# Alexander-H-Liu/End-to-end-ASR-Pytorch

Hardware: AMD Instinct MI355X
Metric: audio frames/sec training (LAS+CTC, LibriSpeech 80-mel) (higher is better)
Workload: dtype f32; 1 GPU; cfg3: {"B": 32, "T": 1600, "D": 80, "V": 5000, "L": 64}; global_batch=32, parallelism=dp1

## Files before the change

### end-to-end-asr-pytorch_amd/csrc/core.cpp

```cpp
#include "common.h"
#include "knobs.h"
#include <cstdlib>
#include <mutex>
#include <vector>

namespace {
struct DevInfo {
    int cu_count = 0;
    int lds_per_cu = 0;
    bool ok = false;
};
DevInfo g_dev[64];

struct ProfRec {
    hipEvent_t a, b;
    int id;
};
bool g_prof_on = false;
std::vector<ProfRec> g_pending;
double g_total_ms[PROF_NUM];
int64_t g_launches[PROF_NUM];
std::mutex g_mu;
hipEvent_t g_cur[PROF_NUM];
}

namespace {
AsrkKnobs g_knobs;
std::once_flag g_knobs_once;
int env_int(const char *name) {
    const char *e = getenv(name);
    return e ? atoi(e) : AsrkKnobs::UNSET;
}
int env_present(const char *name) { return getenv(name) ? 1 : AsrkKnobs::UNSET; }
void read_knobs() {
    AsrkKnobs &k = g_knobs;
    k.gemm_noskinny = env_present("ASRK_GEMM_NOSKINNY");
    k.skinny_sk = env_int("ASRK_SKINNY_SK");
    k.gemm_dbg = env_int("ASRK_GEMM_DBG");
    k.gemm_nofast = env_present("ASRK_GEMM_NOFAST");
    k.split_w256 = env_int("ASRK_SPLIT_W256");
    k.split_tail = env_int("ASRK_SPLIT_TAIL");
    k.split_mfma = env_int("ASRK_SPLIT_MFMA");
    k.fwd_mt = env_int("ASRK_FWD_MT");
    k.fwd_nt = env_int("ASRK_FWD_NT");
    k.rec_bf_mt4 = env_int("ASRK_REC_BF_MT4");
    k.bwd_ub = env_int("ASRK_BWD_UB");
    k.bwd_nt = env_int("ASRK_BWD_NT");
    k.fwd_poll = env_int("ASRK_FWD_POLL");
    k.fwd_presleep = env_int("ASRK_FWD_PRESLEEP");
    k.bwd_poll = env_int("ASRK_BWD_POLL");
    k.bwd_presleep = env_int("ASRK_BWD_PRESLEEP");
    k.dbg_noload = env_present("ASRK_DBG_NOLOAD");
    k.deterministic = env_int("ASRK_DETERMINISTIC");
}
}

const AsrkKnobs &asrk_knobs_() {
    std::call_once(g_knobs_once, read_knobs);
    return g_knobs;
}

extern "C" int asrk_version(void) { return 200; }

extern "C" const char *asrk_strerror(int rc) {
    switch (rc) {
        case ASRK_OK: return "ok";
        case ASRK_EINVAL: return "asrk: invalid argument";
        case ASRK_ESHAPE: return "asrk: shape not supported by the persistent gfx950 kernels";
        case ASRK_EWORKSPACE: return "asrk: workspace too small";
        case ASRK_EDEVICE: return "asrk: device lacks the CUs/LDS the persistent kernel needs";
        case ASRK_ETIMEOUT: return "asrk: in-kernel grid synchronisation timed out";
        default: break;
    }
    if (rc > 0) return hipGetErrorString((hipError_t)rc);
    return "asrk: unknown error";
}

extern "C" int asrk_init(int device) {
    if (device < 0 || device >= 64) return ASRK_EINVAL;
    (void)asrk_knobs_();
    if (!g_dev[device].ok) {
        hipDeviceProp_t prop;
        hipError_t e = hipGetDeviceProperties(&prop, device);
        if (e != hipSuccess) return (int)e > 0 ? -(1000 + (int)e) : ASRK_EDEVICE;
        g_dev[device].cu_count = prop.multiProcessorCount;
        g_dev[device].lds_per_cu = (int)prop.maxSharedMemoryPerMultiProcessor;
        g_dev[device].ok = true;
    }
    return g_dev[device].cu_count;
}

extern "C" int asrk_cu_count_(void) {
    int dev = 0;
    if (hipGetDevice(&dev) != hipSuccess) return 0;
    if (dev < 0 || dev >= 64) return 0;
    if (!g_dev[dev].ok) {
        if (asrk_init(dev) <= 0) return 0;
    }
    return g_dev[dev].cu_count;
}

static double g_work[PROF_NUM] = {0};

static unsigned g_prof_mask = 0xffffffffu;
extern "C" void asrk_profile_enable(int on) { g_prof_on = on != 0; }
extern "C" void asrk_profile_families(unsigned mask) { g_prof_mask = mask; }
static inline bool prof_live(int id) { return g_prof_on && id >= 0 && id < PROF_NUM && ((g_prof_mask >> id) & 1u); }

extern "C" void asrk_profile_reset(void) {
    std::lock_guard<std::mutex> lk(g_mu);
    for (auto &r : g_pending) {
        hipEventDestroy(r.a);
        hipEventDestroy(r.b);
    }
    g_pending.clear();
    for (int i = 0; i < PROF_NUM; ++i) {
        g_total_ms[i] = 0.0;
        g_launches[i] = 0;
        g_work[i] = 0.0;
    }
}

extern "C" void asrk_prof_work_(int id, double flops) {
    if (prof_live(id)) g_work[id] += flops;
}
extern "C" int asrk_profile_get_work(int id, double *flops) {
    if (id < 0 || id >= PROF_NUM || !flops) return ASRK_EINVAL;
    *flops = g_work[id];
    return ASRK_OK;
}

extern "C" void asrk_prof_begin_(int id, hipStream_t s) {
    if (!prof_live(id)) return;
    hipEvent_t a;
    if (hipEventCreate(&a) != hipSuccess) return;
    hipEventRecord(a, s);
    g_cur[id] = a;
}

extern "C" void asrk_prof_end_(int id, hipStream_t s) {
    if (!prof_live(id)) return;
    hipEvent_t b;
    if (hipEventCreate(&b) != hipSuccess) return;
    hipEventRecord(b, s);
    std::lock_guard<std::mutex> lk(g_mu);
    g_pending.push_back({g_cur[id], b, id});
}

extern "C" void asrk_prof_launches_(int id, int64_t n) {
    if (!prof_live(id)) return;
    std::lock_guard<std::mutex> lk(g_mu);
    g_launches[id] += n;
}

extern "C" int asrk_profile_get(int id, double *total_ms, int64_t *launches) {
    if (id < 0 || id >= PROF_NUM) return ASRK_EINVAL;
    std::lock_guard<std::mutex> lk(g_mu);
    for (auto &r : g_pending) {
        hipEventSynchronize(r.b);
        float ms = 0.f;
        if (hipEventElapsedTime(&ms, r.a, r.b) == hipSuccess) {
            g_total_ms[r.id] += ms;
            g_launches[r.id] += 1;
        }
        hipEventDestroy(r.a);
        hipEventDestroy(r.b);
    }
    g_pending.clear();
    if (total_ms) *total_ms = g_total_ms[id];
    if (launches) *launches = g_launches[id];
    return ASRK_OK;
}
```

### end-to-end-asr-pytorch_amd/csrc/gemm_split.hip

```cpp
#include "common.h"
#include "knobs.h"
#include <algorithm>
#include <climits>

extern "C" int asrk_cu_count_(void);

namespace {

typedef __bf16 bf16x8 __attribute__((ext_vector_type(8)));

constexpr int PIECE = 1024;

struct SplitGemmArgs {
    const unsigned char *Ap, *Bp;
    float *C;
    const float *bias, *bias2;
    int M, N, ldc;
    int KC;
    size_t rb_stride_a, rb_stride_b;
    int nk;
    int tiles_m, tiles_n;
    float alpha, beta;
    int slices, ldw;
    float *ws;
};

__device__ __forceinline__ void split8(const float (&v)[8], u32x4 (&w)[3]) {
    unsigned h[3][8];
#pragma unroll
    for (int e = 0; e < 8; ++e) {
        const float a = v[e];
        const __bf16 b0 = (__bf16)a;
        const float r1 = a - (float)b0;
        const __bf16 b1 = (__bf16)r1;
        const float r2 = r1 - (float)b1;
        const __bf16 b2 = (__bf16)r2;
        h[0][e] = __builtin_bit_cast(unsigned short, b0);
        h[1][e] = __builtin_bit_cast(unsigned short, b1);
        h[2][e] = __builtin_bit_cast(unsigned short, b2);
    }
#pragma unroll
    for (int p = 0; p < 3; ++p)
#pragma unroll
        for (int q = 0; q < 4; ++q) w[p][q] = h[p][2 * q] | (h[p][2 * q + 1] << 16);
}

template <bool VEC>
__global__ __launch_bounds__(256) void split_panel_kernel(const float *__restrict__ src, int ld, int R, int K,
                                                          unsigned char *__restrict__ dst, int KC, int RB,
                                                          size_t rb_stride) {
    constexpr int CHUNK = 3 * PIECE;
    const int lane = threadIdx.x & 63;
    const int KG = KC >> 2;
    const int64_t item = (int64_t)blockIdx.x * 4 + (threadIdx.x >> 6);
    if (item >= (int64_t)RB * KG) return;
    const int rb = (int)(item / KG), c0 = (int)(item - (int64_t)rb * KG) * 4;
    unsigned char *drb = dst + (size_t)rb * rb_stride;
    const int c = c0 + (lane & 3), k0 = c * 8;
#pragma unroll
    for (int it = 0; it < 4; ++it) {
        const int rl = it * 16 + (lane >> 2), row = rb * 64 + rl;
        float v[8];
        const float *s = src + (size_t)row * ld + k0;
        if (VEC && row < R && k0 + 8 <= K) {
            const f32x4 lo = *reinterpret_cast<const f32x4 *>(s), hi = *reinterpret_cast<const f32x4 *>(s + 4);
            v[0] = lo[0]; v[1] = lo[1]; v[2] = lo[2]; v[3] = lo[3];
            v[4] = hi[0]; v[5] = hi[1]; v[6] = hi[2]; v[7] = hi[3];
        } else {
#pragma unroll
            for (int e = 0; e < 8; ++e) v[e] = (row < R && k0 + e < K) ? s[e] : 0.f;
        }
        u32x4 w[3];
        split8(v, w);
        unsigned char *d = drb + (size_t)c * CHUNK + rl * 16;
#pragma unroll
        for (int p = 0; p < 3; ++p) *reinterpret_cast<u32x4 *>(d + p * PIECE) = w[p];
    }
}

template <int NCG>
__global__ __launch_bounds__(256) void split_panel_t_kernel(const float *__restrict__ src, int ld, int R, int K,
                                                            unsigned char *__restrict__ dst, int KC, int RB,
                                                            size_t rb_stride) {
    constexpr int CHUNK = 3 * PIECE;
    const int lane = threadIdx.x & 63, wave = __builtin_amdgcn_readfirstlane(threadIdx.x >> 6);
    const int64_t item = (int64_t)blockIdx.x * 4 + wave;
    const int KGn = KC / NCG;
    if (item >= (int64_t)RB * KGn) return;
    const int g = (int)(item / RB), rb = (int)(item - (int64_t)g * RB);
    const int c0 = g * NCG, k0 = c0 * 8, row = rb * 64 + lane;
    float v[NCG][8];
    const float *s = src + (size_t)k0 * ld + row;
    if (k0 + 8 * NCG <= K && rb * 64 + 64 <= R) {
#pragma unroll
        for (int cc = 0; cc < NCG; ++cc)
#pragma unroll
            for (int e = 0; e < 8; ++e) v[cc][e] = s[(size_t)(cc * 8 + e) * ld];
    } else {
#pragma unroll
        for (int cc = 0; cc < NCG; ++cc)
#pragma unroll
            for (int e = 0; e < 8; ++e)
                v[cc][e] = (row < R && k0 + cc * 8 + e < K) ? s[(size_t)(cc * 8 + e) * ld] : 0.f;
    }
    unsigned char *d = dst + (size_t)rb * rb_stride + (size_t)c0 * CHUNK + lane * 16;
#pragma unroll
    for (int cc = 0; cc < NCG; ++cc) {
        u32x4 w[3];
        split8(v[cc], w);
#pragma unroll
        for (int p = 0; p < 3; ++p) *reinterpret_cast<u32x4 *>(d + (size_t)cc * CHUNK + p * PIECE) = w[p];
    }
}

template <int N>
__device__ __forceinline__ void glds16_run(const unsigned char *g, unsigned voff, unsigned char *l) {
    static_assert(N >= 1 && N <= 4, "immediate offset range");
    const auto *gp = (const __attribute__((address_space(1))) unsigned char *)g + voff;
    auto *lp = (__attribute__((address_space(3))) void *)l;
    __builtin_amdgcn_global_load_lds(gp, lp, 16, 0, 0);
    if constexpr (N > 1) __builtin_amdgcn_global_load_lds(gp, lp, 16, PIECE, 0);
    if constexpr (N > 2) __builtin_amdgcn_global_load_lds(gp, lp, 16, 2 * PIECE, 0);
    if constexpr (N > 3) __builtin_amdgcn_global_load_lds(gp, lp, 16, 3 * PIECE, 0);
}

template <int N>
__device__ __forceinline__ void wait_vm() {
    static_assert(N >= 0 && N < 64, "vmcnt is a 6-bit field");
    __builtin_amdgcn_s_waitcnt((N & 15) | 0x70 | 0xF00 | (((N >> 4) & 3) << 14));
}
__device__ __forceinline__ void wait_lgkm0() { __builtin_amdgcn_s_waitcnt(0xC07F); }

template <int NC, int NST, bool SPEC, int WM, bool SK = false>
__global__ __launch_bounds__(SPEC ? (WM == 2 ? 512 : 704) : 256) void gemm_bf16x6_kernel(SplitGemmArgs p) {
    extern __shared__ __attribute__((aligned(1024))) unsigned char lds[];
    static_assert(WM == 2 || (WM == 4 && SPEC), "256-row tiles only with DMA waves");
    static_assert(!SK || NST >= 2, "the split-K epilogue transposes through a stage the last k-tile does not use");
    constexpr int NPL = 3, CHUNK = NPL * PIECE;
    constexpr int NCW = 2 * WM;
    constexpr int NRG = WM + 2;
    constexpr int RPD = WM == 2 ? 1 : 2;
    constexpr int REGION = NC * CHUNK;
    constexpr int STAGE = NRG * REGION;
    constexpr int LPT = NC * NPL * RPD;
    const int tid = threadIdx.x, lane = tid & 63;
    const int wave = __builtin_amdgcn_readfirstlane(tid >> 6);
    const int ntiles = p.tiles_m * p.tiles_n;
    const int slice = SK ? blockIdx.x / ntiles : 0, bid = SK ? blockIdx.x - slice * ntiles : blockIdx.x;
    const int kt0 = SK ? (int)((long)slice * p.nk / p.slices) : 0;
    const int nk = SK ? (int)((long)(slice + 1) * p.nk / p.slices) - kt0 : p.nk;
    const int q8 = ntiles >> 3, r8 = ntiles & 7, xcd = bid & 7, loc = bid >> 3;
    const int tile = (xcd < r8 ? xcd * (q8 + 1) : r8 * (q8 + 1) + (xcd - r8) * q8) + loc;
    constexpr int BAND = 8;
    const int band = tile / (BAND * p.tiles_m);
    const int band_w = min(BAND, p.tiles_n - band * BAND);
    const int in_band = tile - band * BAND * p.tiles_m;
    const int tm = in_band / band_w, tn = band * BAND + in_band % band_w;

    const bool loader = !SPEC || wave >= NCW, worker = !SPEC || wave < NCW;
    const int wr = worker ? wave >> 1 : 0, wc = wave & 1;
    const int ltm = tm, ltn = tn;
    const int r0 = (SPEC ? wave - NCW : wave) * RPD;
    const unsigned char *gsrc[RPD];
#pragma unroll
    for (int q = 0; q < RPD; ++q) {
        const int r = r0 + q;
        gsrc[q] = (r < WM ? p.Ap + (size_t)(ltm * WM + r) * p.rb_stride_a
                          : p.Bp + (size_t)(ltn * 2 + r - WM) * p.rb_stride_b);
        if (SK) gsrc[q] += (size_t)kt0 * REGION;
    }
    const unsigned voff = lane * 16;
    unsigned char *ldst = lds + r0 * REGION;
    static_assert((NC * NPL) % 4 == 0, "a region is issued as runs of four pieces");
    auto issue = [&](int kt, int stage) {
        unsigned char *l = ldst + stage * STAGE;
#pragma unroll
        for (int q = 0; q < RPD; ++q) {
// ... 247 lines not shown
            if (++stage == NST) stage = 0;
        }
        return;
    }

    const int wr = wave >> 1, wc = wave & 1;
    f32x16 acc[2][4];
#pragma unroll
    for (int i = 0; i < 2; ++i)
#pragma unroll
        for (int j = 0; j < 4; ++j)
#pragma unroll
            for (int r = 0; r < 16; ++r) acc[i][j][r] = 0.f;
    const int frag_off = ((lane >> 5) * NPL) * PIECE + (lane & 31) * 16;
    const unsigned char *abase = lds + wr * REGION + frag_off;
    const unsigned char *bbase = lds + (2 + wc * 2) * REGION + frag_off;
    bf16x8 fa1[2], fa2[2], fb1[4], fb2[4], fa0[2][2], fb0[2][4];
    auto rd_a1 = [&](bf16x8 &dst, int stage, int pl, int i) {
        dst = *reinterpret_cast<const bf16x8 *>(abase + stage * STAGE + pl * PIECE + i * 512);
    };
    auto rd_b1 = [&](bf16x8 &dst, int stage, int pl, int j) {
        dst = *reinterpret_cast<const bf16x8 *>(bbase + stage * STAGE + (j >> 1) * REGION + pl * PIECE + (j & 1) * 512);
    };
    auto rd_a = [&](bf16x8 (&dst)[2], int stage, int pl) {
#pragma unroll
        for (int i = 0; i < 2; ++i) rd_a1(dst[i], stage, pl, i);
    };
    auto rd_b = [&](bf16x8 (&dst)[4], int stage, int pl) {
#pragma unroll
        for (int j = 0; j < 4; ++j) rd_b1(dst[j], stage, pl, j);
    };
#define ASRK_TERM8(FA, FB)                                                                                 \
    do {                                                                                                   \
        _Pragma("unroll") for (int i = 0; i < 2; ++i) _Pragma("unroll") for (int j = 0; j < 4; ++j)         \
            acc[i][j] = __builtin_amdgcn_mfma_f32_32x32x16_bf16(FA[i], FB[j], acc[i][j], 0, 0, 0);          \
        __builtin_amdgcn_sched_barrier(0);                                                                 \
    } while (0)
#define ASRK_TERM8_RD(FA, FB, RD)                                                                          \
    do {                                                                                                   \
        _Pragma("unroll") for (int m = 0; m < 8; ++m) {                                                    \
            acc[m >> 2][m & 3] =                                                                           \
                __builtin_amdgcn_mfma_f32_32x32x16_bf16(FA[m >> 2], FB[m & 3], acc[m >> 2][m & 3], 0, 0, 0); \
            __builtin_amdgcn_sched_barrier(0);                                                             \
            RD(m);                                                                                         \
            __builtin_amdgcn_sched_barrier(0);                                                             \
        }                                                                                                  \
    } while (0)
#define ASRK_STEP(P)                                                                                       \
    do {                                                                                                   \
        int nstage = stage + 1;                                                                            \
        if (nstage == NST) nstage = 0;                                                                     \
        ASRK_TERM8(fa2, fb0[P]);                                                                           \
        wait_lgkm0();                                                                                      \
        __builtin_amdgcn_s_barrier();                                           \
        auto rd2 = [&](int m) {                                                                            \
            if (m == 0) rd_a1(fa2[0], nstage, 2, 0);                                                       \
            else if (m == 2) rd_a1(fa2[1], nstage, 2, 1);                                                  \
            else if (m == 4) rd_b1(fb0[1 - (P)][0], nstage, 0, 0);                                         \
            else if (m == 6) rd_b1(fb0[1 - (P)][1], nstage, 0, 1);                                         \
        };                                                                                                 \
        ASRK_TERM8_RD(fa0[P], fb2, rd2);                                                                   \
        auto rd3 = [&](int m) {                                                                            \
            if ((m & 1) == 0) rd_b1(fb2[m >> 1], nstage, 2, m >> 1);                                       \
        };                                                                                                 \
        ASRK_TERM8_RD(fa0[P], fb1, rd3);                                                                   \
        auto rd4 = [&](int m) {                                                                            \
            if (m == 0) rd_b1(fb0[1 - (P)][2], nstage, 0, 2);                                              \
            else if (m == 2) rd_b1(fb0[1 - (P)][3], nstage, 0, 3);                                         \
            else if (m == 4) rd_a1(fa0[1 - (P)][0], nstage, 0, 0);                                         \
            else if (m == 6) rd_a1(fa0[1 - (P)][1], nstage, 0, 1);                                         \
        };                                                                                                 \
        ASRK_TERM8_RD(fa1, fb1, rd4);                                                                      \
        auto rd5 = [&](int m) {                                                                            \
            if ((m & 1) == 0) rd_b1(fb1[m >> 1], nstage, 1, m >> 1);                                       \
        };                                                                                                 \
        ASRK_TERM8_RD(fa1, fb0[P], rd5);                                                                   \
        auto rd6 = [&](int m) {                                                                            \
            if (m == 1) rd_a1(fa1[0], nstage, 1, 0);                                                       \
            else if (m == 4) rd_a1(fa1[1], nstage, 1, 1);                                                  \
        };                                                                                                 \
        ASRK_TERM8_RD(fa0[P], fb0[P], rd6);                                                                \
        stage = nstage;                                                                                    \
    } while (0)

    __builtin_amdgcn_s_barrier();
    rd_a(fa2, 0, 2); rd_b(fb0[0], 0, 0); rd_a(fa0[0], 0, 0); rd_b(fb2, 0, 2); rd_b(fb1, 0, 1); rd_a(fa1, 0, 1);
    int stage = 0;
    for (int kt = 0; kt < nk; kt += 2) {
        ASRK_STEP(0);
        ASRK_STEP(1);
    }
#undef ASRK_STEP
#undef ASRK_TERM8_RD
#undef ASRK_TERM8

    const int row0 = tm * 128 + wr * 64 + 4 * (lane >> 5), col0 = tn * 256 + wc * 128 + (lane & 31);
#pragma unroll
    for (int j = 0; j < 4; ++j) {
        const int col = col0 + j * 32;
        if (col >= p.N) continue;
        float bsum = 0.f;
        if (p.bias) bsum += p.bias[col];
        if (p.bias2) bsum += p.bias2[col];
#pragma unroll
        for (int i = 0; i < 2; ++i)
#pragma unroll
            for (int r = 0; r < 16; ++r) {
                const int row = row0 + i * 32 + (r & 3) + 8 * (r >> 2);
                if (row >= p.M) continue;
                float *c = p.C + (size_t)row * p.ldc + col;
                float v = p.alpha * acc[i][j][r] + bsum;
                if (p.beta != 0.f) v += p.beta * *c;
                *c = v;
            }
    }
}

template <int NST, int NDW>
int launch_split_gemm_w256(const SplitGemmArgs &a, int rb_b, hipStream_t s) {
    constexpr int lds = NST * 6 * 2 * 3 * PIECE;
    auto kern = gemm_bf16x6_w256_kernel<NST, NDW>;
    static AsrkLdsLatch latch;
    ASRK_HIP(asrk_max_lds_once(latch, reinterpret_cast<const void *>(kern), lds));
    const int band = 2;
    hipLaunchKernelGGL(kern, dim3(a.tiles_m * a.tiles_n), dim3((4 + NDW) * 64), lds, s, a, rb_b, band);
    ASRK_LAUNCH_CHECK();
    return ASRK_OK;
}

#define ASRK_P16(FA, FB, ACC, RD)                                                                          \
    do {                                                                                                   \
        _Pragma("unroll") for (int m = 0; m < 16; ++m) {                                                   \
            ACC[m >> 2][m & 3] =                                                                           \
                __builtin_amdgcn_mfma_f32_16x16x32_bf16(FA[m >> 2], FB[m & 3], ACC[m >> 2][m & 3], 0, 0, 0); \
            __builtin_amdgcn_sched_barrier(0);                                                             \
            RD(m);                                                                                         \
            __builtin_amdgcn_sched_barrier(0);                                                             \
        }                                                                                                  \
    } while (0)

template <int START, int STRIDE>
__device__ __forceinline__ void rd16_at(int m, bf16x8 (&slot)[4], const unsigned char *src) {
    static_assert(START + 3 * STRIDE < 16, "inside one product");
    const int i = (m - START) / STRIDE;
    if (m >= START && i < 4 && START + i * STRIDE == m) slot[i] = *reinterpret_cast<const bf16x8 *>(src + i * 256);
}
__device__ __forceinline__ void rd16_all(bf16x8 (&slot)[4], const unsigned char *src) {
#pragma unroll
    for (int i = 0; i < 4; ++i) slot[i] = *reinterpret_cast<const bf16x8 *>(src + i * 256);
}

template <int P> struct StepSet { static constexpr int value = P; };

template <bool SK>
__global__ __launch_bounds__(512) void gemm_bf16x6_m16_kernel(SplitGemmArgs p) {
    extern __shared__ __attribute__((aligned(1024))) unsigned char lds[];
    constexpr int NPL = 3, NC = 4, NST = 3, CHUNK = NPL * PIECE;
    constexpr int REGION = NC * CHUNK, STAGE = 4 * REGION, LPT = NC * NPL;
    const int tid = threadIdx.x, lane = tid & 63;
    const int wave = __builtin_amdgcn_readfirstlane(tid >> 6);
    const int ntiles = p.tiles_m * p.tiles_n;
    const int slice = SK ? blockIdx.x / ntiles : 0, bid = SK ? blockIdx.x - slice * ntiles : blockIdx.x;
    const int kt0 = SK ? (int)((long)slice * p.nk / p.slices) : 0;
    const int nk = SK ? (int)((long)(slice + 1) * p.nk / p.slices) - kt0 : p.nk;
    const int q8 = ntiles >> 3, r8 = ntiles & 7, xcd = bid & 7, loc = bid >> 3;
    const int tile = (xcd < r8 ? xcd * (q8 + 1) : r8 * (q8 + 1) + (xcd - r8) * q8) + loc;
    constexpr int BAND = 8;
    const int band = tile / (BAND * p.tiles_m);
    const int band_w = min(BAND, p.tiles_n - band * BAND);
    const int in_band = tile - band * BAND * p.tiles_m;
    const int tm = in_band / band_w, tn = band * BAND + in_band % band_w;

    const bool worker = wave < 4;
    const int wr = worker ? wave >> 1 : 0, wc = wave & 1;
    const int r0 = worker ? 0 : wave - 4;
    const unsigned char *gsrc = (r0 < 2 ? p.Ap + (size_t)(tm * 2 + r0) * p.rb_stride_a
                                        : p.Bp + (size_t)(tn * 2 + r0 - 2) * p.rb_stride_b) + (size_t)kt0 * REGION;
    const unsigned voff = lane * 16;
    unsigned char *ldst = lds + r0 * REGION;
    auto issue = [&](int kt, int stage) {
        const unsigned char *g = gsrc + (size_t)kt * REGION;
        unsigned char *l = ldst + stage * STAGE;
#pragma unroll
        for (int j = 0; j < LPT; j += 4) glds16_run<4>(g + j * PIECE, voff, l + j * PIECE);
    };

    f32x4 acc[4][4];
#pragma unroll
    for (int i = 0; i < 4; ++i)
#pragma unroll
        for (int j = 0; j < 4; ++j)
#pragma unroll
            for (int r = 0; r < 4; ++r) acc[i][j][r] = 0.f;
    const int frag_off = ((lane >> 4) * NPL) * PIECE + (lane & 15) * 16;
    const unsigned char *abase = lds + wr * REGION + frag_off;
    const unsigned char *bbase = lds + (2 + wc) * REGION + frag_off;
    bf16x8 fa0[2][4], fa1[4], fa2[4], fb0[4], fb1[4], fb2[4];

    if (!worker) {
#pragma unroll
        for (int s = 0; s < NST; ++s)
            if (s < nk) issue(s, s);
        const int later = min(NST - 1, nk - 1);
        if (later >= 2) wait_vm<2 * LPT>();
        else if (later == 1) wait_vm<LPT>();
        else wait_vm<0>();
    }
    __builtin_amdgcn_s_barrier();
    if (worker) {
        rd16_all(fa0[0], abase); rd16_all(fb2, bbase + 2 * PIECE);
        rd16_all(fa1, abase + PIECE); rd16_all(fb1, bbase + PIECE); rd16_all(fa2, abase + 2 * PIECE);
        __builtin_amdgcn_sched_barrier(0);
    }

    int stage = 0, kt = 0;
    auto step = [&](auto set) {
        constexpr int P = decltype(set)::value, Q = 1 - P;
        int nstage = stage + 1;
        if (nstage == NST) nstage = 0;
        const unsigned char *bc = bbase + stage * STAGE;
        const unsigned char *an = abase + nstage * STAGE, *bn = bbase + nstage * STAGE;
        if (worker) {
            auto rd1 = [&](int m) { rd16_at<0, 4>(m, fb0, bc); };
            ASRK_P16(fa0[P], fb2, acc, rd1);
            auto rd2 = [&](int) {};
            ASRK_P16(fa1, fb1, acc, rd2);
            wait_lgkm0();
        } else {
            if (nk - 2 - kt >= 1) wait_vm<LPT>();
            else wait_vm<0>();
        }
        __builtin_amdgcn_s_barrier();
        if (worker) {
            auto rd3 = [&](int m) { rd16_at<0, 4>(m, fb2, bn + 2 * PIECE); };
            ASRK_P16(fa0[P], fb1, acc, rd3);
            auto rd4 = [&](int m) { rd16_at<0, 4>(m, fa0[Q], an); };
            ASRK_P16(fa2, fb0, acc, rd4);
            auto rd5 = [&](int m) { rd16_at<0, 4>(m, fa2, an + 2 * PIECE); rd16_at<2, 4>(m, fb1, bn + PIECE); };
            ASRK_P16(fa1, fb0, acc, rd5);
            auto rd6 = [&](int m) { rd16_at<0, 2>(m, fa1, an + PIECE); };
            ASRK_P16(fa0[P], fb0, acc, rd6);
        } else if (kt + NST < nk) {
            issue(kt + NST, stage);
        }
        stage = nstage;
        ++kt;
    };
    while (kt < nk) {
        step(StepSet<0>());
        if (kt < nk) step(StepSet<1>());
    }
    if (!worker) return;

    if constexpr (SK) {
        constexpr int PITCH = 68;
        static_assert(4 * 16 * PITCH * 4 <= STAGE, "transposition images fit one stage");
        float *img = reinterpret_cast<float *>(lds) + wave * 16 * PITCH;
        float *wsl = p.ws + (size_t)slice * p.M * p.ldw;
        const int wrow0 = tm * 128 + wr * 64, wcol0 = tn * 128 + wc * 64;
        wait_lgkm0();
#pragma unroll
        for (int i = 0; i < 4; ++i) {
#pragma unroll
            for (int j = 0; j < 4; ++j)
#pragma unroll
                for (int r = 0; r < 4; ++r) img[(4 * (lane >> 4) + r) * PITCH + j * 16 + (lane & 15)] = acc[i][j][r];
            __builtin_amdgcn_fence(__ATOMIC_RELEASE, "wavefront");
            __builtin_amdgcn_wave_barrier();
            __builtin_amdgcn_fence(__ATOMIC_ACQUIRE, "wavefront");
#pragma unroll
            for (int q = 0; q < 4; ++q) {
                const int idx = q * 64 + lane, rl = idx >> 4, c4 = (idx & 15) * 4;
                const f32x4 v = *reinterpret_cast<const f32x4 *>(img + rl * PITCH + c4);
                const int row = wrow0 + i * 16 + rl, col = wcol0 + c4;
                if (row < p.M && col < p.ldw) *reinterpret_cast<f32x4 *>(wsl + (size_t)row * p.ldw + col) = v;
            }
            __builtin_amdgcn_fence(__ATOMIC_RELEASE, "wavefront");
            __builtin_amdgcn_wave_barrier();
            __builtin_amdgcn_fence(__ATOMIC_ACQUIRE, "wavefront");
        }
        return;
    }
    const int row0 = tm * 128 + wr * 64 + 4 * (lane >> 4), col0 = tn * 128 + wc * 64 + (lane & 15);
#pragma unroll
    for (int j = 0; j < 4; ++j) {
        const int col = col0 + j * 16;
        if (col >= p.N) continue;
        float bsum = 0.f;
        if (p.bias) bsum += p.bias[col];
        if (p.bias2) bsum += p.bias2[col];
#pragma unroll
        for (int i = 0; i < 4; ++i)
#pragma unroll
            for (int r = 0; r < 4; ++r) {
                const int row = row0 + i * 16 + r;
                if (row >= p.M) continue;
                float *c = p.C + (size_t)row * p.ldc + col;
                float v = p.alpha * acc[i][j][r] + bsum;
                if (p.beta != 0.f) v += p.beta * *c;
                *c = v;
            }
    }
}

template <int NDW>
__global__ __launch_bounds__((4 + NDW) * 64) void gemm_bf16x6_w256_m16_kernel(SplitGemmArgs p, int rb_b, int BAND) {
    extern __shared__ __attribute__((aligned(1024))) unsigned char lds[];
    constexpr int NPL = 3, NC = 2, CHUNK = NPL * PIECE;
    constexpr int REGION = NC * CHUNK, NRG = 6, STAGE = NRG * REGION, PAIR = 2 * STAGE;
    constexpr int LPT = NRG * NC * NPL / NDW, NRUN = LPT / 3;
    static_assert(LPT * NDW == NRG * NC * NPL && NRUN * 3 == LPT, "36 pieces per stage, runs of three");
    const int tid = threadIdx.x, lane = tid & 63;
    const int wave = __builtin_amdgcn_readfirstlane(tid >> 6);
    const int ntiles = p.tiles_m * p.tiles_n, bid = blockIdx.x;
    const int q8 = ntiles >> 3, r8 = ntiles & 7, xcd = bid & 7, loc = bid >> 3;
    const int tile = (xcd < r8 ? xcd * (q8 + 1) : r8 * (q8 + 1) + (xcd - r8) * q8) + loc;
    const int band = tile / (BAND * p.tiles_m);
    const int band_w = min(BAND, p.tiles_n - band * BAND);
    const int in_band = tile - band * BAND * p.tiles_m;
    const int tm = in_band / band_w, tn = band * BAND + in_band % band_w;
    const int ns = p.nk >> 1;

    const bool worker = wave < 4;
    const int first = (worker ? 0 : wave - 4) * LPT;
    const unsigned char *run_g[NRUN];
#pragma unroll
    for (int k = 0; k < NRUN; ++k) {
        const int idx = first + 3 * k, r = idx / (NC * NPL), j = idx - r * (NC * NPL);
        run_g[k] = (r < 2 ? p.Ap + (size_t)(tm * 2 + r) * p.rb_stride_a
                          : p.Bp + (size_t)min(tn * 4 + r - 2, rb_b - 1) * p.rb_stride_b) + j * PIECE;
    }
    const unsigned voff = lane * 16;
    unsigned char *ldst = lds + first * PIECE;
    auto issue_pair = [&](int s, int slot) {
#pragma unroll
        for (int h = 0; h < 2; ++h) {
            unsigned char *l = ldst + slot * PAIR + h * STAGE;
            const size_t gk = (size_t)(2 * s + h) * REGION;
#pragma unroll
            for (int k = 0; k < NRUN; ++k) glds16_run<3>(run_g[k] + gk, voff, l + 3 * k * PIECE);
        }
    };

    const int wr = worker ? wave >> 1 : 0, wc = wave & 1;
    f32x4 acc0[4][4], acc1[4][4];
#pragma unroll
    for (int i = 0; i < 4; ++i)
#pragma unroll
        for (int j = 0; j < 4; ++j)
#pragma unroll
            for (int r = 0; r < 4; ++r) acc0[i][j][r] = acc1[i][j][r] = 0.f;
    const int frag_off = (lane >> 5) * STAGE + (((lane >> 4) & 1) * NPL) * PIECE + (lane & 15) * 16;
    const unsigned char *abase = lds + wr * REGION + frag_off;
    const unsigned char *bbase = lds + (2 + wc * 2) * REGION + frag_off;
    bf16x8 fa0[2][4], fa1[4], fa2[4], fb0[4], fb1[4], fb2[4];

    if (!worker) {
        issue_pair(0, 0);
        if (ns > 1) {
            issue_pair(1, 1);
            wait_vm<2 * LPT>();
        } else {
            wait_vm<0>();
        }
    }
    __builtin_amdgcn_s_barrier();
    if (worker) {
        rd16_all(fa0[0], abase); rd16_all(fb2, bbase + 2 * PIECE);
        rd16_all(fa1, abase + PIECE); rd16_all(fb1, bbase + PIECE); rd16_all(fa2, abase + 2 * PIECE);
        __builtin_amdgcn_sched_barrier(0);
    }

    int s = 0;
    auto step = [&](auto set) {
        constexpr int P = decltype(set)::value, Q = 1 - P;
        const unsigned char *bc = bbase + P * PAIR;
        const unsigned char *an = abase + Q * PAIR, *bn = bbase + Q * PAIR;
        auto rd0 = [&](int) {};
        if (worker) {
            auto rd1 = [&](int m) { rd16_at<0, 4>(m, fb0, bc); };
            ASRK_P16(fa0[P], fb2, acc0, rd1);
            auto rd2 = [&](int m) { rd16_at<0, 4>(m, fb2, bc + REGION + 2 * PIECE); };
            ASRK_P16(fa1, fb1, acc0, rd2);
            ASRK_P16(fa0[P], fb1, acc0, rd0);
            auto rd4 = [&](int m) { rd16_at<0, 4>(m, fb1, bc + REGION + PIECE); };
            ASRK_P16(fa2, fb0, acc0, rd4);
            ASRK_P16(fa1, fb0, acc0, rd0);
            ASRK_P16(fa0[P], fb0, acc0, rd0);
            wait_lgkm0();
            auto rd7 = [&](int m) { rd16_at<0, 4>(m, fb0, bc + REGION); };
            ASRK_P16(fa0[P], fb2, acc1, rd7);
            ASRK_P16(fa1, fb1, acc1, rd0);
            wait_lgkm0();
        } else {
            wait_vm<0>();
        }
        __builtin_amdgcn_s_barrier();
        if (worker) {
            auto rd9 = [&](int m) { rd16_at<0, 4>(m, fb2, bn + 2 * PIECE); };
            ASRK_P16(fa0[P], fb1, acc1, rd9);
            auto rd10 = [&](int m) { rd16_at<0, 4>(m, fa0[Q], an); };
            ASRK_P16(fa2, fb0, acc1, rd10);
            auto rd11 = [&](int m) { rd16_at<0, 4>(m, fa2, an + 2 * PIECE); rd16_at<2, 4>(m, fb1, bn + PIECE); };
            ASRK_P16(fa1, fb0, acc1, rd11);
            auto rd12 = [&](int m) { rd16_at<0, 2>(m, fa1, an + PIECE); };
            ASRK_P16(fa0[P], fb0, acc1, rd12);
        } else if (s + 2 < ns) {
            issue_pair(s + 2, P);
        }
        ++s;
    };
    while (s < ns) {
        step(StepSet<0>());
        if (s < ns) step(StepSet<1>());
    }
    if (!worker) return;

    const int row0 = tm * 128 + wr * 64 + 4 * (lane >> 4), col0 = tn * 256 + wc * 128 + (lane & 15);
#pragma unroll
    for (int j = 0; j < 8; ++j) {
        const int col = col0 + j * 16;
        if (col >= p.N) continue;
        float bsum = 0.f;
        if (p.bias) bsum += p.bias[col];
        if (p.bias2) bsum += p.bias2[col];
#pragma unroll
        for (int i = 0; i < 4; ++i)
#pragma unroll
            for (int r = 0; r < 4; ++r) {
                const int row = row0 + i * 16 + r;
                if (row >= p.M) continue;
                float *c = p.C + (size_t)row * p.ldc + col;
                float v = p.alpha * (j < 4 ? acc0[i][j & 3][r] : acc1[i][j & 3][r]) + bsum;
                if (p.beta != 0.f) v += p.beta * *c;
                *c = v;
            }
    }
}
#undef ASRK_P16

template <bool SK>
int launch_split_gemm_m16(const SplitGemmArgs &a, hipStream_t s) {
    constexpr int lds = 3 * 4 * 4 * 3 * PIECE;
    auto kern = gemm_bf16x6_m16_kernel<SK>;
    static AsrkLdsLatch latch;
    ASRK_HIP(asrk_max_lds_once(latch, reinterpret_cast<const void *>(kern), lds));
    hipLaunchKernelGGL(kern, dim3(a.tiles_m * a.tiles_n * (SK ? a.slices : 1)), dim3(512), lds, s, a);
    ASRK_LAUNCH_CHECK();
    if (SK) {
        const int64_t items = (int64_t)a.M * (a.ldw >> 2);
        hipLaunchKernelGGL(splitk_reduce_kernel, dim3((unsigned)asrk_div_up64(items, 256)), dim3(256), 0, s, a.ws,
                           a.slices, a.M, a.N, a.ldw, a.alpha, a.beta, a.C, a.ldc, a.bias, a.bias2);
        ASRK_LAUNCH_CHECK();
    }
    return ASRK_OK;
}

int launch_split_gemm_w256_m16(const SplitGemmArgs &a, int rb_b, hipStream_t s) {
    constexpr int lds = 4 * 6 * 2 * 3 * PIECE;
    auto kern = gemm_bf16x6_w256_m16_kernel<4>;
    static AsrkLdsLatch latch;
    ASRK_HIP(asrk_max_lds_once(latch, reinterpret_cast<const void *>(kern), lds));
    const int band = 2;
    hipLaunchKernelGGL(kern, dim3(a.tiles_m * a.tiles_n), dim3(512), lds, s, a, rb_b, band);
    ASRK_LAUNCH_CHECK();
    return ASRK_OK;
}

template <int NC, int NST, bool SPEC, int WM, bool SK = false>
int launch_split_gemm(const SplitGemmArgs &a, hipStream_t s) {
    constexpr int lds = NST * (WM + 2) * NC * 3 * PIECE;
    auto kern = gemm_bf16x6_kernel<NC, NST, SPEC, WM, SK>;
    static AsrkLdsLatch latch;
    ASRK_HIP(asrk_max_lds_once(latch, reinterpret_cast<const void *>(kern), lds));
    hipLaunchKernelGGL(kern, dim3(a.tiles_m * a.tiles_n * (SK ? a.slices : 1)), dim3(SPEC ? (WM == 2 ? 512 : 704) : 256),
                       lds, s, a);
    ASRK_LAUNCH_CHECK();
    if (SK) {
        const int64_t items = (int64_t)a.M * (a.ldw >> 2);
        hipLaunchKernelGGL(splitk_reduce_kernel, dim3((unsigned)asrk_div_up64(items, 256)), dim3(256), 0, s, a.ws,
                           a.slices, a.M, a.N, a.ldw, a.alpha, a.beta, a.C, a.ldc, a.bias, a.bias2);
        ASRK_LAUNCH_CHECK();
    }
    return ASRK_OK;
}

}

namespace {
constexpr int SPLIT_NC = 4;
constexpr int NPL = 3;
constexpr int SPLIT_MFMA16_MIN_NK = 48;

struct PanelGeom {
    int KC, rb;
    size_t rb_stride, bytes;
};
PanelGeom panel_geom(int rows, int K, bool slack = false) {
    PanelGeom g;
    g.KC = (asrk_div_up(K, 8 * SPLIT_NC) + (slack ? 1 : 0)) * SPLIT_NC;
    g.rb = asrk_div_up(rows, 128) * 2;
    g.rb_stride = (size_t)g.KC * NPL * PIECE + 4352;
    g.bytes = (size_t)g.rb * g.rb_stride;
    return g;
}

int run_split(const float *src, int ld, int rows, int K, bool trans, unsigned char *dstp, const PanelGeom &g,
              hipStream_t s) {
    const dim3 grid((unsigned)asrk_div_up64((int64_t)g.rb * (g.KC / 4), 4));
    asrk_prof_work_(PROF_SPLIT, 4.0 * (double)rows * (double)K + 6.0 * (double)g.rb * 64.0 * (double)g.KC * 8.0);
    asrk_prof_begin_(PROF_SPLIT, s);
    if (trans) {
        hipLaunchKernelGGL((split_panel_t_kernel<4>), grid, dim3(256), 0, s, src, ld, rows, K, dstp, g.KC, g.rb, g.rb_stride);
    } else {
        const bool vec = (reinterpret_cast<uintptr_t>(src) & 15) == 0 && ld % 4 == 0;
        if (vec) hipLaunchKernelGGL((split_panel_kernel<true>), grid, dim3(256), 0, s, src, ld, rows, K, dstp, g.KC, g.rb, g.rb_stride);
        else hipLaunchKernelGGL((split_panel_kernel<false>), grid, dim3(256), 0, s, src, ld, rows, K, dstp, g.KC, g.rb, g.rb_stride);
    }
    asrk_prof_end_(PROF_SPLIT, s);
    ASRK_LAUNCH_CHECK();
    return ASRK_OK;
}

int auto_slices(int M, int N, int nk) {
    if (N >= 512) return 1;
    const int ncu = asrk_cu_count_() > 0 ? asrk_cu_count_() : 256;
    const long tiles = (long)asrk_div_up(M, 128) * asrk_div_up(N, 128);
    const long want = (ncu + tiles - 1) / tiles;
    return (int)std::max(1L, std::min(want, (long)(nk / 64)));
}

int run_panel_gemm(int M, int N, int nk, float alpha, const unsigned char *Ap, size_t stride_a,
                   const unsigned char *Bp, size_t stride_b, float beta, float *C, int ldc, const float *bias,
                   const float *bias2, hipStream_t s, int slices = 1, float *ws = nullptr) {
    const AsrkKnobs &kn = asrk_knobs_();
    SplitGemmArgs a;
    a.Ap = Ap; a.Bp = Bp; a.C = C; a.bias = bias; a.bias2 = bias2;
    a.M = M; a.N = N; a.ldc = ldc; a.KC = 0; a.nk = nk; a.rb_stride_a = stride_a; a.rb_stride_b = stride_b;
    a.tiles_m = asrk_div_up(M, 128); a.tiles_n = asrk_div_up(N, 128);
    a.alpha = alpha; a.beta = beta;
    a.slices = std::min(slices, nk); a.ldw = (N + 3) & ~3; a.ws = ws;
    const bool m16 = kn.is_set(kn.split_mfma) ? kn.split_mfma == 16 : nk >= SPLIT_MFMA16_MIN_NK;
    const bool m16_sk = kn.is_set(kn.split_mfma) && kn.split_mfma == 16;
    const bool m16_128 = m16, m16_w256 = m16;
    if (a.slices > 1) return m16_sk ? launch_split_gemm_m16<true>(a, s) : launch_split_gemm<4, 3, true, 2, true>(a, s);
    const int w256 = kn.get(kn.split_w256, 1);
    if (w256 && N >= 512) {
        const int tm = asrk_div_up(M, 128), tn = asrk_div_up(N, 256);
        const int ncu = asrk_cu_count_() > 0 ? asrk_cu_count_() : 256;
        if (w256 == 2 || (long)tm * tn >= 2L * ncu) {
            SplitGemmArgs b = a;
            b.tiles_m = tm; b.tiles_n = tn; b.nk = 2 * nk;
            const long tiles = (long)tm * tn, rem = tiles % ncu;
            const int tm1 = (int)((tiles - rem) / tn);
            if (w256 == 1 && rem > 0 && rem * 10 < 6L * ncu && tm1 > 0 && tm1 < tm && kn.get(kn.split_tail, 1)) {
                b.tiles_m = tm1; b.M = tm1 * 128;
                int rc = m16_w256 ? launch_split_gemm_w256_m16(b, 2 * asrk_div_up(N, 128), s)
                                  : launch_split_gemm_w256<4, 4>(b, 2 * asrk_div_up(N, 128), s);
                if (rc != ASRK_OK) return rc;
                SplitGemmArgs c = a;
                c.Ap = a.Ap + (size_t)tm1 * 2 * a.rb_stride_a;
                c.C = a.C + (size_t)tm1 * 128 * ldc;
                c.M = M - tm1 * 128;
                c.tiles_m = asrk_div_up(c.M, 128);
                return m16_128 ? launch_split_gemm_m16<false>(c, s) : launch_split_gemm<4, 3, true, 2>(c, s);
            }
            return m16_w256 ? launch_split_gemm_w256_m16(b, 2 * asrk_div_up(N, 128), s)
                            : launch_split_gemm_w256<4, 4>(b, 2 * asrk_div_up(N, 128), s);
        }
    }
    return m16_128 ? launch_split_gemm_m16<false>(a, s) : launch_split_gemm<4, 3, true, 2>(a, s);
}
}

extern "C" size_t asrk_split_panel_stride_(int rows, int K) { return panel_geom(rows, K, true).rb_stride; }

extern "C" int asrk_gemm_takes_split(int M, int N, int K, int flags) {
    const int mode = flags & 3;
    if (mode == ASRK_GEMM_SPLIT_OFF || mode == 3 || K < 8 || M < 1 || N < 1) return 0;
    if (mode == ASRK_GEMM_SPLIT_AUTO) {
        const double hm = 2.0 * (double)M * (double)N / ((double)M + (double)N);
        const bool shallow_ok = K >= 64 && (double)M * (double)N >= 134217728.0;
        if (hm < 1500.0 || (K < 256 && !shallow_ok) || M < 256 || N < 256) return 0;
    }
    return 1;
}

extern "C" size_t asrk_gemm_ws_bytes(int M, int N, int K, int flags) {
    if (!asrk_gemm_takes_split(M, N, K, flags)) return 0;
    return panel_geom(M, K).bytes + panel_geom(N, K).bytes;
}

extern "C" int asrk_gemm_split_run_(int transA, int transB, int M, int N, int K, float alpha, const float *A,
                                    int lda, const float *B, int ldb, float beta, float *C, int ldc,
                                    const float *bias, const float *bias2, void *wsp, int flags, hipStream_t s) {
    const PanelGeom ga = panel_geom(M, K), gb = panel_geom(N, K);
    unsigned char *ws = reinterpret_cast<unsigned char *>(wsp);
    unsigned char *Ap = ws, *Bp = ws + ga.bytes;
    int rc = run_split(A, lda, M, K, transA != 0, Ap, ga, s);
    if (rc != ASRK_OK) return rc;
    rc = run_split(B, ldb, N, K, transB == 0, Bp, gb, s);
    if (rc != ASRK_OK) return rc;
    return run_panel_gemm(M, N, ga.KC / SPLIT_NC, alpha, Ap, ga.rb_stride, Bp, gb.rb_stride, beta, C, ldc, bias,
                          bias2, s);
}

extern "C" size_t asrk_split_panel_bytes(int rows, int K, int flags) {
    if (rows <= 0 || K <= 0 || flags != 0) return 0;
    return panel_geom(rows, K, true).bytes;
}

extern "C" int asrk_split_panel_f32(const float *src, int ld, int rows, int K, int trans, void *panel, int flags,
                                    void *stream) {
    if (!src || !panel || rows <= 0 || K <= 0 || ld < (trans ? rows : K) || flags != 0) return ASRK_EINVAL;
    if ((reinterpret_cast<uintptr_t>(panel) & 15) != 0) return ASRK_EINVAL;
    asrk_prof_begin_(PROF_GEMM, (hipStream_t)stream);
    const int rc = run_split(src, ld, rows, K, trans != 0, reinterpret_cast<unsigned char *>(panel),
                             panel_geom(rows, K, true), (hipStream_t)stream);
    asrk_prof_end_(PROF_GEMM, (hipStream_t)stream);
    return rc;
}

namespace {
struct PanelRange {
    const unsigned char *Ap, *Bp;
    size_t stride_a, stride_b;
    int nk;
};
int panel_range(int M, int N, int K, const void *A_panel, int a_rows, int a_K, int a_row0, int a_k0,
                const void *B_panel, int b_rows, int b_K, int b_row0, int b_k0, const float *C, int ldc, int flags,
                PanelRange &r) {
    if (M <= 0 || N <= 0 || K <= 0 || !A_panel || !B_panel || !C || ldc < N || flags != 0) return ASRK_EINVAL;
    if (a_row0 < 0 || b_row0 < 0 || a_k0 < 0 || b_k0 < 0 || a_row0 % 128 || b_row0 % 128 || a_k0 % 8 || b_k0 % 8)
        return ASRK_EINVAL;
    if (a_row0 + M > a_rows || b_row0 + N > b_rows || a_k0 + K > a_K || b_k0 + K > b_K) return ASRK_EINVAL;
    if (K % 32 != 0 && a_k0 + K != a_K && b_k0 + K != b_K) return ASRK_ESHAPE;
    const PanelGeom ga = panel_geom(a_rows, a_K, true), gb = panel_geom(b_rows, b_K, true);
    r.nk = asrk_div_up(K, 32);
    if (a_k0 / 8 + r.nk * SPLIT_NC > ga.KC || b_k0 / 8 + r.nk * SPLIT_NC > gb.KC) return ASRK_ESHAPE;
    const unsigned char *A0 = reinterpret_cast<const unsigned char *>(A_panel);
    const unsigned char *B0 = reinterpret_cast<const unsigned char *>(B_panel);
    r.Ap = A0 + (size_t)(a_row0 / 64) * ga.rb_stride + (size_t)(a_k0 / 8) * NPL * PIECE;
    r.Bp = B0 + (size_t)(b_row0 / 64) * gb.rb_stride + (size_t)(b_k0 / 8) * NPL * PIECE;
    r.stride_a = ga.rb_stride; r.stride_b = gb.rb_stride;
    return ASRK_OK;
}
}

extern "C" int asrk_gemm_panels_f32(int M, int N, int K, float alpha, const void *A_panel, int a_rows, int a_K,
                                    int a_row0, int a_k0, const void *B_panel, int b_rows, int b_K, int b_row0,
                                    int b_k0, float beta, float *C, int ldc, const float *bias,
                                    const float *bias2, int flags, void *stream) {
    PanelRange r;
    const int rc0 = panel_range(M, N, K, A_panel, a_rows, a_K, a_row0, a_k0, B_panel, b_rows, b_K, b_row0, b_k0, C, ldc,
                                flags, r);
    if (rc0 != ASRK_OK) return rc0;
    hipStream_t s = (hipStream_t)stream;
    asrk_prof_work_(PROF_GEMM, 2.0 * (double)M * (double)N * (double)K);
    asrk_prof_begin_(PROF_GEMM, s);
    const int rc = run_panel_gemm(M, N, r.nk, alpha, r.Ap, r.stride_a, r.Bp, r.stride_b, beta, C, ldc, bias, bias2, s);
    asrk_prof_end_(PROF_GEMM, s);
    return rc;
}

extern "C" size_t asrk_gemm_panels_splitk_ws_bytes(int M, int N, int splitk) {
    if (M <= 0 || N <= 0 || splitk < 0) return 0;
    const int n = splitk > 0 ? splitk : auto_slices(M, N, INT_MAX);
    return (size_t)n * (size_t)M * (size_t)((N + 3) & ~3) * sizeof(float);
}

extern "C" int asrk_gemm_panels_splitk_f32(int M, int N, int K, float alpha, const void *A_panel, int a_rows, int a_K,
                                           int a_row0, int a_k0, const void *B_panel, int b_rows, int b_K,
                                           int b_row0, int b_k0, float beta, float *C, int ldc, const float *bias,
                                           const float *bias2, int splitk, void *ws, size_t ws_bytes, int flags,
                                           void *stream) {
    if (splitk < 0 || !ws || (reinterpret_cast<uintptr_t>(ws) & 15) != 0) return ASRK_EINVAL;
    PanelRange r;
    const int rc0 = panel_range(M, N, K, A_panel, a_rows, a_K, a_row0, a_k0, B_panel, b_rows, b_K, b_row0, b_k0, C, ldc,
                                flags, r);
    if (rc0 != ASRK_OK) return rc0;
    const int slices = splitk > 0 ? splitk : auto_slices(M, N, r.nk);
    if (ws_bytes < asrk_gemm_panels_splitk_ws_bytes(M, N, slices)) return ASRK_EWORKSPACE;
    hipStream_t s = (hipStream_t)stream;
    asrk_prof_work_(PROF_GEMM, 2.0 * (double)M * (double)N * (double)K);
    asrk_prof_begin_(PROF_GEMM, s);
    const int rc = run_panel_gemm(M, N, r.nk, alpha, r.Ap, r.stride_a, r.Bp, r.stride_b, beta, C, ldc, bias, bias2, s,
                                  slices, reinterpret_cast<float *>(ws));
    asrk_prof_end_(PROF_GEMM, s);
    return rc;
}
```

### end-to-end-asr-pytorch_amd/csrc/knobs.h

```cpp
#pragma once

struct AsrkKnobs {
    static constexpr int UNSET = -0x7fffffff;
    int gemm_noskinny;
    int skinny_sk;
    int gemm_dbg;
    int gemm_nofast;
    int split_w256;
    int split_tail;
    int split_mfma;
    int fwd_mt, fwd_nt;
    int rec_bf_mt4;
    int bwd_ub, bwd_nt;
    int fwd_poll, fwd_presleep;
    int bwd_poll, bwd_presleep;
    int dbg_noload;
    int deterministic;

    int get(int v, int dflt) const { return v == UNSET ? dflt : v; }
    bool is_set(int v) const { return v != UNSET; }
};

const AsrkKnobs &asrk_knobs_();
```

Before: 552,400 frames/s.

## Add thin-K persistent GEMM kernel and LDS-staged coalesced epilogue for split GEMMs

```diff
diff --git a/end-to-end-asr-pytorch_amd/csrc/core.cpp b/end-to-end-asr-pytorch_amd/csrc/core.cpp
--- a/end-to-end-asr-pytorch_amd/csrc/core.cpp
+++ b/end-to-end-asr-pytorch_amd/csrc/core.cpp
@@ -41,6 +41,8 @@
     k.split_w256 = env_int("ASRK_SPLIT_W256");
     k.split_tail = env_int("ASRK_SPLIT_TAIL");
     k.split_mfma = env_int("ASRK_SPLIT_MFMA");
+    k.split_think = env_int("ASRK_SPLIT_THINK");
+    k.split_epi = env_int("ASRK_SPLIT_EPI");
     k.fwd_mt = env_int("ASRK_FWD_MT");
     k.fwd_nt = env_int("ASRK_FWD_NT");
     k.rec_bf_mt4 = env_int("ASRK_REC_BF_MT4");
diff --git a/end-to-end-asr-pytorch_amd/csrc/gemm_split.hip b/end-to-end-asr-pytorch_amd/csrc/gemm_split.hip
--- a/end-to-end-asr-pytorch_amd/csrc/gemm_split.hip
+++ b/end-to-end-asr-pytorch_amd/csrc/gemm_split.hip
@@ -23,6 +23,7 @@
     float alpha, beta;
     int slices, ldw;
     float *ws;
+    int epi, vec;
 };
 
 __device__ __forceinline__ void split8(const float (&v)[8], u32x4 (&w)[3]) {
@@ -576,6 +577,47 @@
 
 template <int P> struct StepSet { static constexpr int value = P; };
 
+template <int NJ, typename F>
+__device__ __forceinline__ void m16_strip_store(float *img, F &&val, const float (&bsum)[NJ], const SplitGemmArgs &p,
+                                                int row_base, int col_base, int lane) {
+    constexpr int W = NJ * 16, PITCH = W + 4, LPR = W / 4;
+#pragma unroll
+    for (int j = 0; j < NJ; ++j)
+#pragma unroll
+        for (int r = 0; r < 4; ++r)
+            img[(4 * (lane >> 4) + r) * PITCH + j * 16 + (lane & 15)] = p.alpha * val(j, r) + bsum[j];
+    __builtin_amdgcn_fence(__ATOMIC_RELEASE, "wavefront");
+    __builtin_amdgcn_wave_barrier();
+    __builtin_amdgcn_fence(__ATOMIC_ACQUIRE, "wavefront");
+#pragma unroll
+    for (int q = 0; q < 16 * LPR / 64; ++q) {
+        const int idx = q * 64 + lane, rl = idx / LPR, c4 = (idx % LPR) * 4;
+        f32x4 v = *reinterpret_cast<const f32x4 *>(img + rl * PITCH + c4);
+        const int row = row_base + rl, col = col_base + c4;
+        if (row >= p.M) continue;
+        float *c = p.C + (size_t)row * p.ldc + col;
+        if (p.vec && col + 4 <= p.N) {
+            if (p.beta != 0.f) {
+                const f32x4 c0 = *reinterpret_cast<const f32x4 *>(c);
+#pragma unroll
+                for (int e = 0; e < 4; ++e) v[e] += p.beta * c0[e];
+            }
+            *reinterpret_cast<f32x4 *>(c) = v;
+        } else {
+#pragma unroll
+            for (int e = 0; e < 4; ++e) {
+                if (col + e >= p.N) break;
+                float o = v[e];
+                if (p.beta != 0.f) o += p.beta * c[e];
+                c[e] = o;
+            }
+        }
+    }
+    __builtin_amdgcn_fence(__ATOMIC_RELEASE, "wavefront");
+    __builtin_amdgcn_wave_barrier();
+    __builtin_amdgcn_fence(__ATOMIC_ACQUIRE, "wavefront");
+}
+
 template <bool SK>
 __global__ __launch_bounds__(512) void gemm_bf16x6_m16_kernel(SplitGemmArgs p) {
     extern __shared__ __attribute__((aligned(1024))) unsigned char lds[];
@@ -703,6 +745,25 @@
             __builtin_amdgcn_wave_barrier();
             __builtin_amdgcn_fence(__ATOMIC_ACQUIRE, "wavefront");
         }
+        return;
+    }
+    if (p.epi) {
+        float *img = reinterpret_cast<float *>(lds) + wave * 16 * 68;
+        float bsum[4];
+#pragma unroll
+        for (int j = 0; j < 4; ++j) {
+            const int col = tn * 128 + wc * 64 + j * 16 + (lane & 15);
+            bsum[j] = 0.f;
+            if (col < p.N) {
+                if (p.bias) bsum[j] += p.bias[col];
+                if (p.bias2) bsum[j] += p.bias2[col];
+            }
+        }
+        wait_lgkm0();
+#pragma unroll
+        for (int i = 0; i < 4; ++i)
+            m16_strip_store<4>(img, [&](int j, int r) { return acc[i][j][r]; }, bsum, p, tm * 128 + wr * 64 + i * 16,
+                               tn * 128 + wc * 64, lane);
         return;
     }
     const int row0 = tm * 128 + wr * 64 + 4 * (lane >> 4), col0 = tn * 128 + wc * 64 + (lane & 15);
@@ -840,6 +901,26 @@
     }
     if (!worker) return;
 
+    if (p.epi) {
+        float *img = reinterpret_cast<float *>(lds) + wave * 16 * 132;
+        static_assert(4 * 16 * 132 * 4 <= STAGE, "strip images fit one stage");
+        float bsum[8];
+#pragma unroll
+        for (int j = 0; j < 8; ++j) {
+            const int col = tn * 256 + wc * 128 + j * 16 + (lane & 15);
+            bsum[j] = 0.f;
+            if (col < p.N) {
+                if (p.bias) bsum[j] += p.bias[col];
+                if (p.bias2) bsum[j] += p.bias2[col];
+            }
+        }
+        wait_lgkm0();
+#pragma unroll
+        for (int i = 0; i < 4; ++i)
+            m16_strip_store<8>(img, [&](int j, int r) { return j < 4 ? acc0[i][j & 3][r] : acc1[i][j & 3][r]; }, bsum, p,
+                               tm * 128 + wr * 64 + i * 16, tn * 256 + wc * 128, lane);
+        return;
+    }
     const int row0 = tm * 128 + wr * 64 + 4 * (lane >> 4), col0 = tn * 256 + wc * 128 + (lane & 15);
 #pragma unroll
     for (int j = 0; j < 8; ++j) {
@@ -889,6 +970,167 @@
     hipLaunchKernelGGL(kern, dim3(a.tiles_m * a.tiles_n), dim3(512), lds, s, a, rb_b, band);
     ASRK_LAUNCH_CHECK();
     return ASRK_OK;
+}
+
+constexpr int THINK_PITCH = 132;
+constexpr int THINK_IMG = 8 * THINK_PITCH * 4;
+constexpr int THINK_MAX_NK = 4;
+
+template <int NK>
+__global__ __launch_bounds__(512) void gemm_bf16x6_think_kernel(SplitGemmArgs p, int nslice, int nrange) {
+    extern __shared__ __attribute__((aligned(1024))) unsigned char lds[];
+    constexpr int NPL = 3, CHUNK = NPL * PIECE, NS = 2 * NK;
+    constexpr int BREG = NK * 4 * CHUNK;
+    const int tid = threadIdx.x, lane = tid & 63;
+    const int wave = __builtin_amdgcn_readfirstlane(tid >> 6);
+    const int nwg = nslice * nrange, bid = blockIdx.x;
+    const int q8 = nwg >> 3, r8 = nwg & 7, xcd = bid & 7, loc = bid >> 3;
+    const int w = (xcd < r8 ? xcd * (q8 + 1) : r8 * (q8 + 1) + (xcd - r8) * q8) + loc;
+    const int range = w / nslice, slice = w - range * nslice;
+    const int items = (p.M + 31) >> 5;
+    const int it0 = (int)((long)range * items / nrange), it1 = (int)((long)(range + 1) * items / nrange);
+
+    const unsigned lane_off = (lane >> 5) * CHUNK + (lane & 31) * 16;
+    auto a_ptr = [&](int it) { return p.Ap + (size_t)(it >> 1) * p.rb_stride_a + (it & 1) * 512 + lane_off; };
+    bf16x8 fa[NS][NPL];
+    int it = it0 + wave;
+    if (it < it1) {
+        const unsigned char *g = a_ptr(it);
+#pragma unroll
+        for (int s = 0; s < NS; ++s)
+#pragma unroll
+            for (int pl = 0; pl < NPL; ++pl)
+                fa[s][pl] = *reinterpret_cast<const bf16x8 *>(g + (s * 2 * NPL + pl) * PIECE);
+    }
+#pragma unroll
+    for (int rb = 0; rb < 2; ++rb) {
+        const unsigned char *g = p.Bp + (size_t)(slice * 2 + rb) * p.rb_stride_b;
+        for (int off = tid * 16; off < BREG; off += 512 * 16)
+            *reinterpret_cast<u32x4 *>(lds + rb * BREG + off) = *reinterpret_cast<const u32x4 *>(g + off);
+    }
+    __syncthreads();
+    if (it >= it1) return;
+
+    const unsigned char *bbase = lds + lane_off;
+    auto rd_b = [&](int s, int pl, int j) {
+        return *reinterpret_cast<const bf16x8 *>(bbase + (j >> 1) * BREG + (j & 1) * 512 + (s * 2 * NPL + pl) * PIECE);
+    };
+    float *img = reinterpret_cast<float *>(lds + 2 * BREG + wave * THINK_IMG);
+    float bsum[4];
+#pragma unroll
+    for (int j = 0; j < 4; ++j) {
+        const int col = slice * 128 + j * 32 + (lane & 31);
+        bsum[j] = 0.f;
+        if (col < p.N) {
+            if (p.bias) bsum[j] += p.bias[col];
+            if (p.bias2) bsum[j] += p.bias2[col];
+        }
+    }
+    bf16x8 fb0[2][4], fb1[4], fb2[4];
+#pragma unroll
+    for (int j = 0; j < 4; ++j) {
+        fb0[0][j] = rd_b(0, 0, j);
+        fb2[j] = rd_b(0, 2, j);
+        fb1[j] = rd_b(0, 1, j);
+    }
+    f32x16 acc[4];
+#define ASRK_TK(FA, FB, RD)                                                                                \
+    do {                                                                                                   \
+        _Pragma("unroll") for (int j = 0; j < 4; ++j) {                                                    \
+            acc[j] = __builtin_amdgcn_mfma_f32_32x32x16_bf16(FA, FB[j], acc[j], 0, 0, 0);                  \
+            __builtin_amdgcn_sched_barrier(0);                                                             \
+            RD(j);                                                                                         \
+            __builtin_amdgcn_sched_barrier(0);                                                             \
+        }                                                                                                  \
+    } while (0)
+    for (; it < it1; it += 8) {
+#pragma unroll
+        for (int j = 0; j < 4; ++j)
+#pragma unroll
+            for (int r = 0; r < 16; ++r) acc[j][r] = 0.f;
+        const unsigned char *gn = a_ptr(it + 8 < it1 ? it + 8 : it);
+#pragma unroll
+        for (int s = 0; s < NS; ++s) {
+            const int P = s & 1, Q = P ^ 1, sn = s + 1 == NS ? 0 : s + 1;
+            auto rd_none = [&](int) {};
+            auto rd_b0 = [&](int j) { fb0[Q][j] = rd_b(sn, 0, j); };
+            auto rd_b2 = [&](int j) { fb2[j] = rd_b(sn, 2, j); };
+            auto rd_b1 = [&](int j) { fb1[j] = rd_b(sn, 1, j); };
+            ASRK_TK(fa[s][2], fb0[P], rd_none);
+            ASRK_TK(fa[s][0], fb2, rd_b0);
+            ASRK_TK(fa[s][0], fb1, rd_b2);
+            ASRK_TK(fa[s][1], fb1, rd_none);
+            ASRK_TK(fa[s][1], fb0[P], rd_b1);
+            ASRK_TK(fa[s][0], fb0[P], rd_none);
+#pragma unroll
+            for (int pl = 0; pl < NPL; ++pl)
+                fa[s][pl] = *reinterpret_cast<const bf16x8 *>(gn + (s * 2 * NPL + pl) * PIECE);
+            __builtin_amdgcn_sched_barrier(0);
+        }
+        const int row0 = it * 32;
+#pragma unroll
+        for (int g = 0; g < 4; ++g) {
+#pragma unroll
+            for (int j = 0; j < 4; ++j)
+#pragma unroll
+                for (int rr = 0; rr < 4; ++rr)
+                    img[(rr + 4 * (lane >> 5)) * THINK_PITCH + j * 32 + (lane & 31)] = p.alpha * acc[j][4 * g + rr] + bsum[j];
+            __builtin_amdgcn_fence(__ATOMIC_RELEASE, "wavefront");
+            __builtin_amdgcn_wave_barrier();
+            __builtin_amdgcn_fence(__ATOMIC_ACQUIRE, "wavefront");
+#pragma unroll
+            for (int q = 0; q < 4; ++q) {
+                const int idx = q * 64 + lane, rl = idx >> 5, c4 = (idx & 31) * 4;
+                f32x4 v = *reinterpret_cast<const f32x4 *>(img + rl * THINK_PITCH + c4);
+                const int row = row0 + 8 * g + rl, col = slice * 128 + c4;
+                if (row >= p.M) continue;
+                float *c = p.C + (size_t)row * p.ldc + col;
+                if (p.vec && col + 4 <= p.N) {
+                    if (p.beta != 0.f) {
+                        const f32x4 c0 = *reinterpret_cast<const f32x4 *>(c);
+#pragma unroll
+                        for (int e = 0; e < 4; ++e) v[e] += p.beta * c0[e];
+                    }
+                    *reinterpret_cast<f32x4 *>(c) = v;
+                } else {
+#pragma unroll
+                    for (int e = 0; e < 4; ++e) {
+                        if (col + e >= p.N) break;
+                        float o = v[e];
+                        if (p.beta != 0.f) o += p.beta * c[e];
+                        c[e] = o;
+                    }
+                }
+            }
+            __builtin_amdgcn_fence(__ATOMIC_RELEASE, "wavefront");
+            __builtin_amdgcn_wave_barrier();
+            __builtin_amdgcn_fence(__ATOMIC_ACQUIRE, "wavefront");
+        }
+    }
+#undef ASRK_TK
+}
+
+template <int NK>
+int launch_split_gemm_think(const SplitGemmArgs &a, hipStream_t s) {
+    constexpr int lds = 2 * NK * 4 * 3 * PIECE + 8 * THINK_IMG;
+    auto kern = gemm_bf16x6_think_kernel<NK>;
+    static AsrkLdsLatch latch;
+    ASRK_HIP(asrk_max_lds_once(latch, reinterpret_cast<const void *>(kern), lds));
+    const int ncu = asrk_cu_count_() > 0 ? asrk_cu_count_() : 256;
+    const int nslice = asrk_div_up(a.N, 128), items = asrk_div_up(a.M, 32);
+    const int nrange = std::max(1, std::min(items, ncu / nslice));
+    hipLaunchKernelGGL(kern, dim3(nslice * nrange), dim3(512), lds, s, a, nslice, nrange);
+    ASRK_LAUNCH_CHECK();
+    return ASRK_OK;
+}
+
+int launch_split_gemm_think_nk(const SplitGemmArgs &a, hipStream_t s) {
+    switch (a.nk) {
+    case 1: return launch_split_gemm_think<1>(a, s);
+    case 2: return launch_split_gemm_think<2>(a, s);
+    case 3: return launch_split_gemm_think<3>(a, s);
+    default: return launch_split_gemm_think<4>(a, s);
+    }
 }
 
 template <int NC, int NST, bool SPEC, int WM, bool SK = false>
@@ -915,6 +1157,7 @@
 constexpr int SPLIT_NC = 4;
 constexpr int NPL = 3;
 constexpr int SPLIT_MFMA16_MIN_NK = 48;
+constexpr int SPLIT_EPI_DEFAULT = 1;
 
 struct PanelGeom {
     int KC, rb;
@@ -964,10 +1207,18 @@
     a.tiles_m = asrk_div_up(M, 128); a.tiles_n = asrk_div_up(N, 128);
     a.alpha = alpha; a.beta = beta;
     a.slices = std::min(slices, nk); a.ldw = (N + 3) & ~3; a.ws = ws;
+    a.epi = kn.get(kn.split_epi, SPLIT_EPI_DEFAULT);
+    a.vec = (reinterpret_cast<uintptr_t>(C) & 15) == 0 && ldc % 4 == 0;
     const bool m16 = kn.is_set(kn.split_mfma) ? kn.split_mfma == 16 : nk >= SPLIT_MFMA16_MIN_NK;
     const bool m16_sk = kn.is_set(kn.split_mfma) && kn.split_mfma == 16;
     const bool m16_128 = m16, m16_w256 = m16;
     if (a.slices > 1) return m16_sk ? launch_split_gemm_m16<true>(a, s) : launch_split_gemm<4, 3, true, 2, true>(a, s);
+    const int think = kn.get(kn.split_think, 1);
+    if (think && nk <= THINK_MAX_NK && !m16_sk) {
+        const int ncu = asrk_cu_count_() > 0 ? asrk_cu_count_() : 256;
+        if (think == 2 || (N >= 512 && (long)asrk_div_up(M, 128) * asrk_div_up(N, 256) >= 2L * ncu))
+            return launch_split_gemm_think_nk(a, s);
+    }
     const int w256 = kn.get(kn.split_w256, 1);
     if (w256 && N >= 512) {
         const int tm = asrk_div_up(M, 128), tn = asrk_div_up(N, 256);
diff --git a/end-to-end-asr-pytorch_amd/csrc/knobs.h b/end-to-end-asr-pytorch_amd/csrc/knobs.h
--- a/end-to-end-asr-pytorch_amd/csrc/knobs.h
+++ b/end-to-end-asr-pytorch_amd/csrc/knobs.h
@@ -9,6 +9,8 @@
     int split_w256;
     int split_tail;
     int split_mfma;
+    int split_think;
+    int split_epi;
     int fwd_mt, fwd_nt;
     int rec_bf_mt4;
     int bwd_ub, bwd_nt;
```

Result: no change. 555,500 frames/s (median of 6 runs) (+0.6%).
